# UM-Applied-Algorithms-Lab/AWRY

Measured on AMD Instinct MI355X. Metric: k-mer count queries/sec (parallel_count, random 31-mers, index resident in HBM), higher is better.
Workload: dtype u64

## Files before the change

awry_amd/_lib.py:

```python
import ctypes as C
import importlib.util
import os
import re

_HERE = os.path.dirname(os.path.abspath(__file__))
_SO = os.path.join(_HERE, "lib", "libawry_hip.so")
_HEADER = os.path.join(os.path.dirname(_HERE), "include", "awry_hip.h")
_lib = None


def lib_path():
    return _SO


class Pos(C.Structure):
    _fields_ = [("seq_idx", C.c_uint64), ("local_pos", C.c_uint64)]


class Range(C.Structure):
    _fields_ = [("start_ptr", C.c_uint64), ("end_ptr", C.c_uint64)]


class Anchor(C.Structure):
    _fields_ = [("q_begin", C.c_uint32), ("q_len", C.c_uint32), ("start_row", C.c_uint64), ("count", C.c_uint64)]
# ... 57 lines not shown

def load_library():
    global _lib
    if _lib is not None:
        return _lib
    if not os.path.exists(_SO):
        raise ImportError(
            "libawry_hip.so is not built (%s).  Run `python -m awry_amd.build` (needs hipcc); "
            "there is no CPU fallback for the search path." % _SO)
    _preload_hip_runtime()
    L = C.CDLL(_SO)
    vp, u64, u8, i32, cp = C.c_void_p, C.c_uint64, C.c_uint8, C.c_int, C.c_char_p
    u64p, u8p = C.POINTER(C.c_uint64), C.POINTER(C.c_uint8)
    vpp = C.POINTER(vp)

    def sig(name, res, *args):
        f = getattr(L, name)
        f.restype, f.argtypes = res, list(args)

    sig("awry_last_error", cp)
    sig("awry_build", i32, C.POINTER(BuildArgs), vpp)
    sig("awry_build_from_text", i32, vp, u64, i32, u64, u8, u64p, C.POINTER(cp), u64, vpp)
    sig("awry_build_from_text_on", i32, vp, u64, i32, u64, u8, u64p, C.POINTER(cp), u64, i32, vpp)
    sig("awry_load", i32, cp, vpp)
    sig("awry_save", i32, vp, cp)
    sig("awry_free", None, vp)
    sig("awry_set_devices", i32, vp, C.POINTER(i32), i32)
    sig("awry_set_seed_kmer_len", i32, vp, i32)
    sig("awry_seed_kmer_len", i32, vp)
    sig("awry_debug_set_count_kernel", i32, i32)
    sig("awry_debug_force_wide_rows", i32, i32)
    sig("awry_debug_set_max_blocks", i32, i32)
    sig("awry_debug_max_blocks", i32)
    sig("awry_debug_dense_sa", vp, vp, i32)
    sig("awry_debug_accelerators", i32, vp, i32, C.POINTER(DebugAccel))
    sig("awry_debug_seed_rung", vp, vp, i32, i32)
    sig("awry_debug_set_ctx_extra_cap", i32, i32)
    sig("awry_count_schedule", cp, vp, i32)
    sig("awry_num_devices", i32, vp)
    sig("awry_replica_device", i32, vp, i32)
    sig("awry_count_batch", i32, vp, vp, u64p, u64, u64p)
    sig("awry_count_packed_kmers", i32, vp, u64p, u64, i32, u64p)
    sig("awry_locate_batch", i32, vp, vp, u64p, u64, C.POINTER(u64p), C.POINTER(C.POINTER(Pos)), C.POINTER(u64p))
    sig("awry_free_buffer", None, vp)
    sig("awry_count_mismatch_batch", i32, vp, vp, u64p, u64, i32, u64p)
    sig("awry_locate_mismatch_batch", i32, vp, vp, u64p, u64, i32, C.POINTER(u64p), C.POINTER(C.POINTER(Pos)), C.POINTER(u64p),
        C.POINTER(u8p))
    sig("awry_dev_count_mismatch", i32, vp, i32, vp, vp, u64, i32, vp, vp, vp)
    sig("awry_dev_count_mismatch_tally", i32, vp, i32, vp, vp, u64, i32, vp, vp, vp, vp)
    u32 = C.c_uint32
    sig("awry_pattern_class", u32, i32, u8)
    sig("awry_count_pattern_batch", i32, vp, vp, u64p, u64, i32, u64p)
    sig("awry_locate_pattern_batch", i32, vp, vp, u64p, u64, i32, C.POINTER(u64p), C.POINTER(C.POINTER(Pos)), C.POINTER(u64p),
        C.POINTER(u8p))
    sig("awry_dev_count_pattern", i32, vp, i32, vp, vp, u64, i32, vp, vp, vp)
    sig("awry_dev_count_pattern_tally", i32, vp, i32, vp, vp, u64, i32, vp, vp, vp, vp)
    app = C.POINTER(C.POINTER(Anchor))
    sig("awry_anchor_batch", i32, vp, vp, u64p, u64, u32, i32, C.POINTER(u64p), app)
    sig("awry_locate_anchors_batch", i32, vp, vp, u64p, u64, u32, i32, u64, C.POINTER(u64p), app, C.POINTER(u64p),
        C.POINTER(C.POINTER(Pos)), C.POINTER(u64p))
    sig("awry_dev_anchors", i32, vp, i32, vp, vp, u64, u32, i32, vp, vp, vp, vp, vp)
    sig("awry_dev_anchors_tally", i32, vp, i32, vp, vp, u64, u32, i32, vp, vp, vp, vp, vp, vp)
    sig("awry_smem_batch", i32, vp, vp, u64p, u64, u32, C.POINTER(u64p), app)
    sig("awry_locate_smems_batch", i32, vp, vp, u64p, u64, u32, u64, C.POINTER(u64p), app, C.POINTER(u64p), C.POINTER(C.POINTER(Pos)), C.POINTER(u64p))
    sig("awry_dev_smems", i32, vp, i32, vp, vp, u64, u32, vp, vp, vp, vp, vp)
    sig("awry_dev_smems_tally", i32, vp, i32, vp, vp, u64, u32, vp, vp, vp, vp, vp, vp)
# ... 96 lines not shown
```

awry_amd/csrc/awry_hip.hip:

```cpp
#include "dev_common.h"
#include "replica.h"
#include "accelerators.h"
#include "launchers.h"
#include "host_count.h"
#include "host_locate.h"
#include "batch_host.h"
#include "mismatch_host.h"
#include "anchor_host.h"
#include "chain_host.h"
#include "edit_host.h"
#include "chain_align_host.h"
#include "map_host.h"
#include "pair_host.h"
#include "prewarm.h"

namespace {

template <class T>
T* malloc_array(size_t n) {
  const size_t bytes = std::max<size_t>(1, n) * sizeof(T);
  void* p = nullptr;
  if (bytes >= (8u << 20)) {
    if (posix_memalign(&p, 2u << 20, bytes) != 0) p = nullptr;
    if (p) (void)madvise(p, bytes, MADV_HUGEPAGE);
// ... 190 lines not shown
    idx->reps.clear();
    std::vector<std::unique_ptr<Replica>> reps(n_devices);
    if (n_devices == 1) {
      reps[0] = make_replica(idx, device_ids[0]);
    } else {
      std::vector<std::exception_ptr> errs(n_devices);
      std::vector<std::thread> pool;
      for (int i = 0; i < n_devices; i++)
        pool.emplace_back([&, i] {
          try { reps[i] = make_replica(idx, device_ids[i]); } catch (...) { errs[i] = std::current_exception(); }
        });
      for (auto& t : pool) t.join();
      for (auto& e : errs) if (e) std::rethrow_exception(e);
    }
    idx->reps = std::move(reps);
    for (auto& r : idx->reps) prewarm_host_paths(*r);
  });
}

int awry_set_seed_kmer_len(awry_index_t* idx, int k) {
  return guarded([&] {
    require(idx != nullptr, "null index");
    require(k >= -1 && k <= 17, "seed k-mer length must be in -1..17 (amino: ..7)");
    idx->seed_k_request = k;
    for (size_t s = 0; s < idx->reps.size(); s++) {
      Replica& r = replica(idx, (int)s);
      build_seed(idx, r, k < 0 ? default_seed_k(idx->host) : k);
      sync_seed_mode(idx, r);
    }
  });
}

int awry_debug_set_count_kernel(int mode) { g_count_kernel.store(mode); return AWRY_OK; }
int awry_debug_force_wide_rows(int on) { g_force_wide.store(on ? 1 : 0); return AWRY_OK; }
int awry_debug_set_max_blocks(int blocks) {
  if (blocks < 0) { g_last_error = "awry_debug_set_max_blocks: negative bound"; return AWRY_ERR_ARG; }
  g_max_blocks.store(blocks);
  return AWRY_OK;
}
int awry_debug_max_blocks(void) { return g_max_blocks.load(); }

const char* awry_count_schedule(const awry_index_t* idx, int L) {
  if (!idx || idx->reps.empty()) return "";
  const CountFacts f = count_facts(*idx->reps[0]);
  const uint64_t n = 1u << 20;
  return plan_name(L > 32 ? plan_reads(f, n, L, true, false) : plan_kmers(f, n, L, true, false));
}

int awry_seed_kmer_len(const awry_index_t* idx) { return idx && !idx->reps.empty() ? idx->reps[0]->seed_k : 0; }
int awry_num_devices(const awry_index_t* idx) { return idx ? (int)idx->reps.size() : 0; }
int awry_replica_device(const awry_index_t* idx, int slot) {
  return idx && slot >= 0 && slot < (int)idx->reps.size() ? idx->reps[slot]->device : -1;
}

int awry_count_batch(awry_index_t* idx, const uint8_t* qbytes, const uint64_t* qoff, uint64_t n, uint64_t* counts_out) {
  return guarded([&] {
    require(idx && qoff && (counts_out || n == 0), "null argument");
    require(qbytes || qoff[n] == qoff[0], "null query bytes");
    const auto t0 = std::chrono::steady_clock::now();
    for_each_replica(idx, n, [&](Replica& r, Shard sh, int) { count_shard(r, qbytes, qoff, sh, counts_out); });
    if (getenv("AWRY_TRACE_HOST"))
      fprintf(stderr, "[awry] awry_count_batch %.2f ms\n", std::chrono::duration<double, std::milli>(std::chrono::steady_clock::now() - t0).count());
  });
}

int awry_count_packed_kmers(awry_index_t* idx, const uint64_t* words, uint64_t n, int L, uint64_t* counts_out) {
// ... 1031 lines not shown
```

awry_amd/csrc/kernels.hip.h:

```cpp
#pragma once
#include <hip/hip_runtime.h>

#include "alphabet.h"
#include "layout.h"

#include "kernels_rank.hip.h"
#include "kernels_scan.hip.h"
#include "kernels_count.hip.h"
#include "kernels_anchor.hip.h"
#include "kernels_smem.hip.h"
#include "kernels_aa_kmer.hip.h"
#include "kernels_quad.hip.h"
#include "lcx.hip.h"
#include "kernels_nt2_kmer.hip.h"
#include "kmer_table.hip.h"
#include "kernels_seed.hip.h"
#include "kernels_pack.hip.h"
#include "kernels_reads.hip.h"
#include "lcx_kernels.hip.h"
#include "kernels_wide.hip.h"

namespace awry {

constexpr int LOC_TILE = 1024;
constexpr int LOC_QCAP = 1024;

constexpr uint64_t LOC_WALK_FLAG = 1ull << 63;

__device__ __forceinline__ void localise(const DevIndex& ix, uint64_t g, uint64_t* __restrict__ out) {
  uint64_t a = 0, z = ix.nseq;
  if (ix.seq_bucket) {
    const uint64_t b = g >> ix.seq_bucket_shift;
    a = ix.seq_bucket[b];
    z = (uint64_t)ix.seq_bucket[b + 1] + 1;
  }
  while (z - a > 1) { uint64_t mid = (a + z) >> 1; if (ix.seq_starts[mid] <= g) a = mid; else z = mid; }
  out[0] = a;
// ... 409 lines not shown
```

awry_amd/csrc/kernels_reads.hip.h:

```cpp
#pragma once

namespace awry {

template <bool USE_SEED, bool VERIFY, bool LIST, bool RAGGED>
__device__ __forceinline__ void reads_body(const DevIndex& ix, const uint64_t* __restrict__ queries, uint64_t n, int L,
                                           uint64_t* __restrict__ counts, uint64_t* __restrict__ range_start,
                                           const uint32_t* __restrict__ list_q, const uint32_t* __restrict__ lens, bool allow_lcx,
                                           uint64_t r_start = ~0ull, uint64_t r_stride = 64) {
  const int l = threadIdx.x & 3;
  const uint64_t nquads = ((uint64_t)gridDim.x * blockDim.x) >> 2;
  uint64_t r = r_start == ~0ull ? threadIdx.x >> 2 : r_start;
  uint64_t q = LIST ? (r < n ? list_q[r] : 0) : ((uint64_t)blockIdx.x * blockDim.x + threadIdx.x) >> 2;
  const uint64_t* __restrict__ blocks = ix.blocks;
  const SeedEntry* __restrict__ seed = ix.seed;
  const uint32_t* __restrict__ dense = ix.dense_sa;
  const uint32_t* __restrict__ text4 = ix.text4;
  const int k = USE_SEED ? ix.seed_k : 1, W = (L + 31) / 32;
  const int verify_after = (int)ix.verify_after;
  const bool lcx = USE_SEED && VERIFY && ix.lcx_key != nullptr && allow_lcx;
  const uint32_t cA = (uint32_t)ix.prefix_sums[1], cC = (uint32_t)ix.prefix_sums[2], cG = (uint32_t)ix.prefix_sums[3],
                 cN = (uint32_t)ix.prefix_sums[4], cT = (uint32_t)ix.prefix_sums[5], cEnd = (uint32_t)ix.prefix_sums[6];
  bool have = LIST ? r < n : q < n, fresh = true;
  uint64_t w = 0;
  uint32_t sp = 1, ep = 0;
// ... 145 lines not shown
          out_count = (uint64_t)__popc(vmask);
          if (ep == sp && vmask) out_rs = (RS_SINGLE << RS_MODE_SHIFT) | ((uint64_t)vp - (uint64_t)i);
          else out_rs = ((cand_lcx ? RS_LCX : RS_MULTI) << RS_MODE_SHIFT) | (uint64_t)sp | ((uint64_t)i << 32) | ((uint64_t)vmask << 48);
          cand_lcx = false;
        }
      }
      if (finished) {
        if (l == 0 && !hole) {
          counts[q] = out_count;
          if (range_start) range_start[q] = out_rs;
        }
        if (LIST) {
          r += r_stride;
          have = r < n;
          q = have ? list_q[r] : 0;
        } else {
          q += nquads;
          have = q < n;
        }
        fresh = true;
        mode = 0;
      }
    }
  }
}

template <bool USE_SEED, bool VERIFY, bool LIST = false, bool RAGGED = false>
__global__ __launch_bounds__(256) void count_nt2_reads_kernel(DevIndex ix, const uint64_t* __restrict__ queries, uint64_t n, int L,
                                                              uint64_t* __restrict__ counts, uint64_t* __restrict__ range_start,
                                                              Nt2Survivors sv = Nt2Survivors{}, const uint32_t* __restrict__ lens = nullptr) {
  if (LIST) reads_body<USE_SEED, VERIFY, LIST, RAGGED>(ix, queries, (uint64_t)sv.count[blockIdx.x], L, counts, range_start, sv.q + (uint64_t)blockIdx.x * sv.cap, lens, true);
  else reads_body<USE_SEED, VERIFY, LIST, RAGGED>(ix, queries, n, L, counts, range_start, nullptr, lens, true);
}
template <bool RAGGED>
__global__ __launch_bounds__(256) void count_nt2_reads_pool_kernel(DevIndex ix, const uint64_t* __restrict__ queries, int L, uint64_t* __restrict__ counts,
                                                                   uint64_t* __restrict__ range_start, Nt2Survivors sv, const uint32_t* __restrict__ lens) {
  reads_body<true, true, true, RAGGED>(ix, queries, (uint64_t)sv.count[0], L, counts, range_start, sv.q, lens, false,
                                       ((uint64_t)blockIdx.x * blockDim.x + threadIdx.x) >> 2, ((uint64_t)gridDim.x * blockDim.x) >> 2);
}

template <bool RAGGED>
__global__ __launch_bounds__(256) void count_nt2_reads_probe_kernel(DevIndex ix, const uint64_t* __restrict__ queries, uint64_t n, int L,
                                                                    uint64_t* __restrict__ counts, uint64_t* __restrict__ range_start,
                                                                    Nt2Survivors sv, const uint32_t* __restrict__ lens) {
  constexpr int VQ = 192;
  __shared__ unsigned int s_count;
  __shared__ uint32_t s_vsp[4][VQ], s_vq[4][VQ];
  __shared__ uint8_t s_vn[4][VQ];
  __shared__ uint16_t s_vl[RAGGED ? 4 : 1][VQ];
  __shared__ uint64_t s_vw[4][3][VQ];
  if (threadIdx.x == 0) s_count = 0;
  if (blockIdx.x == 0 && threadIdx.x == 0 && sv.lf_count) *sv.lf_count = 0;
  __syncthreads();
  const int lane = threadIdx.x & 63, wv_id = threadIdx.x >> 6;
  const SeedEntry* __restrict__ seed = ix.seed;
  const int k = ix.seed_k, W = (L + 31) / 32;
  const bool pos = ix.seed_pos != 0;
  const int min_i0 = pos ? 1 : 3;
  const int cx = (int)ix.ctx_extra, clen = SEED_CTX_LEN + cx;
  const uint64_t kmask = (1ull << (2 * k)) - 1;
  const uint64_t stride = (uint64_t)gridDim.x * blockDim.x;
  const uint64_t lane_lt = (1ull << lane) - 1;
  const uint64_t region = (uint64_t)blockIdx.x * sv.cap;
  const bool stash = L - k <= 96;
  int vcount = 0;
  auto settle = [&](uint64_t q, uint64_t count, uint64_t rs) {
    counts[q] = count;
    if (range_start) range_start[q] = rs;
  };
  auto drain = [&](int base, int cnt) {
    uint32_t q[2], sp[2], nc[2], vp[2];
    bool on[2];
#pragma unroll
    for (int h = 0; h < 2; h++) {
      const int s = base + lane + 64 * h;
      on[h] = lane + 64 * h < cnt;
      q[h] = on[h] ? s_vq[wv_id][s] : 0;
      sp[h] = on[h] ? s_vsp[wv_id][s] : 0;
      nc[h] = on[h] ? s_vn[wv_id][s] : 0;
      vp[h] = on[h] ? ((pos && nc[h] == 1u) ? sp[h] : ix.dense_sa[sp[h]]) : 0;
    }
#pragma unroll
    for (int h = 0; h < 2; h++) {
      if (!on[h]) continue;
      const int i0 = (RAGGED ? (int)s_vl[RAGGED ? wv_id : 0][base + lane + 64 * h] : L) - k, nchunks = (i0 + 31) >> 5;
// ... 125 lines not shown
```

awry_amd/csrc/launchers.h:

```cpp
#pragma once

namespace {

std::atomic<int> g_count_kernel{-1};
int count_kernel_override() {
  int m = g_count_kernel.load();
  if (m >= 0) return m;
  const char* e = getenv("AWRY_COUNT_KERNEL");
  if (e && !strcmp(e, "strided")) return 0;
  if (e && !strcmp(e, "chunk")) return 1;
  if (e && !strcmp(e, "quad4")) return 2;
  if (e && !strcmp(e, "twophase")) return 3;
  return -1;
}

CountFacts count_facts(const Replica& r) {
  static const bool rungs_off = getenv("AWRY_SEED_RUNGS") && !strcmp(getenv("AWRY_SEED_RUNGS"), "0");
  static const bool table_off = getenv("AWRY_KMER_TABLE") && !strcmp(getenv("AWRY_KMER_TABLE"), "0");
  CountFacts f;
  f.alphabet = r.dev.alphabet;
  f.wide = r.wide;
  f.bwt_len = r.dev.bwt_len;
  f.seed_k = r.seed_k;
  f.seed = r.seed.p != nullptr;
  f.seed64 = r.dev.seed64 != nullptr;
  f.text4 = r.dev.text4 != nullptr;
  f.dense_ratio = r.dev.dense_ratio;
  f.lcx_key = r.dev.lcx_key != nullptr;
  f.kt_mode = r.kt_mode;
  f.verify_kmers = r.verify_kmers;
  f.num_cus = r.num_cus;
  for (int i = 0; i < 4; i++) f.probe_resume_per_cu[i] = r.probe_resume_per_cu[i];
  for (int i = 0; i < 2; i++) f.lcx_reads_grid[i] = r.lcx_reads_grid[i];
  f.forced = count_kernel_override();
  f.rungs_off = rungs_off;
  f.table_off = table_off;
  return f;
}
dim3 plan_grid(const Replica& r, const CountPlan& p, uint64_t n) {
  return dim3(p.blocks ? p.blocks : (unsigned)grid_for(r, n * p.items_per_query, 256));
}


void launch_pack_nt2(Replica& r, const uint8_t* d_ascii, const uint64_t* d_off, uint64_t base, uint64_t n, uint64_t total_bytes, int L, int W,
                     uint64_t* d_words, uint32_t* d_lens, unsigned long long* d_bad, hipStream_t s, uint32_t* d_bad_list = nullptr) {
  if (n == 0) return;
// ... 130 lines not shown
    });
  } else {
    require(p.schedule == CountSchedule::WIDE_SINGLE, "internal: not a wide-row schedule");
    with_flags(p.seeded, d_lens != nullptr, [&](auto S, auto R) {
      hipLaunchKernelGGL((count_nt2_wide_kernel<S(), R()>), gw, bw, 0, s, r.dev, d_words, n, L, d_counts, d_range_start, d_lens, d_tally);
    });
  }
  HIP_CHECK(hipGetLastError());
}

void launch_count_nt2_long(Replica& r, const uint64_t* d_words, uint64_t n, int L, uint64_t* d_counts, uint64_t* d_range_start,
                           bool use_seed, hipStream_t s, const uint32_t* d_lens = nullptr) {
  require(r.dev.alphabet == NUCLEOTIDE, "packed 2-bit queries need a nucleotide index");
  require(L >= 1 && L <= 1 << 20, "packed read length out of range");
  if (n == 0) return;
  const ScratchLock scratch_lock(r, s);
  const CountPlan p = plan_reads(count_facts(r), n, L, use_seed, d_lens != nullptr);
  const dim3 g(plan_grid(r, p, n)), b(256);
  switch (p.schedule) {
    case CountSchedule::WIDE_SINGLE:
    case CountSchedule::WIDE_TWO_PHASE:
      launch_count_nt2_wide(r, p, d_words, n, L, d_counts, d_range_start, s, d_lens, nullptr);
      return;
    case CountSchedule::READS_LISTS:
    case CountSchedule::READS_LANES: {
      const bool lanes = p.schedule == CountSchedule::READS_LANES;
      Nt2Survivors sv, fb;
      two_phase_lists(r, s, n, p.blocks, p.lcx_grid, &sv, &fb);
      if (!lanes) sv.w = sv.range = nullptr;
      with_flags(d_lens != nullptr, [&](auto R) {
        hipLaunchKernelGGL(count_nt2_reads_probe_kernel<R()>, g, b, 0, s, r.dev, d_words, n, L, d_counts, d_range_start, sv, d_lens);
        if (lanes) {
          hipLaunchKernelGGL(lcx_quad_reads_kernel<R()>, dim3(p.lcx_grid), b, 0, s, r.dev, d_words, L, d_counts, d_range_start, sv, fb, p.blocks, d_lens);
          hipLaunchKernelGGL(count_nt2_reads_pool_kernel<R()>, g, b, 0, s, r.dev, d_words, L, d_counts, d_range_start, fb, d_lens);
        } else hipLaunchKernelGGL((count_nt2_reads_kernel<true, true, true, R()>), g, b, 0, s, r.dev, d_words, n, L, d_counts, d_range_start, sv, d_lens);
      });
      break;
    }
    case CountSchedule::READS_SINGLE: {
      const Nt2Survivors none{};
      with_flags(p.seeded, p.verify, d_lens != nullptr, [&](auto S, auto V, auto R) {
        hipLaunchKernelGGL((count_nt2_reads_kernel<S(), V(), false, R()>), g, b, 0, s, r.dev, d_words, n, L, d_counts, d_range_start, none, d_lens);
      });
      break;
    }
    default: require(false, "internal: not a schedule for reads");
  }
  HIP_CHECK(hipGetLastError());
}

void launch_count_nt2(Replica& r, const uint64_t* d_words, uint64_t n, int L, uint64_t* d_counts, bool use_seed, hipStream_t s,
                      unsigned long long* d_tally = nullptr) {
  require(r.dev.alphabet == NUCLEOTIDE, "packed 2-bit queries need a nucleotide index");
  require(L >= 1 && L <= 32, "packed k-mer length must be in 1..32");
  if (n == 0) return;
  const ScratchLock scratch_lock(r, s);
  CountFacts f = count_facts(r);
  CountPlan p = plan_kmers(f, n, L, use_seed, d_tally != nullptr);
  DevIndex dv = r.dev;
  std::shared_lock<std::shared_mutex> kt_lock;
  if (p.rung) {
    if (const SeedEntry* t = seed_rung(r, L)) { dv.seed = t; dv.seed_k = L; dv.seed_pos = 0; dv.ctx_extra = 0; }
    else { f.rung_failed = true; p = plan_kmers(f, n, L, use_seed, d_tally != nullptr); }
  }
  if (p.table) {
    if (const Replica::KmerTable* kt = kmer_table(r, L, true, kt_lock)) { dv.kmer_tab = kt->tab.p; dv.kmer_tab_bits = kt->bits; }
    else { f.table_failed = true; p = plan_kmers(f, n, L, use_seed, d_tally != nullptr); }
// ... 348 lines not shown
```

awry_amd/fm_index.py:

```python
import ctypes as C
import os
from dataclasses import dataclass
from typing import Iterable, List, Optional, Sequence

import numpy as np

from . import _lib

NUCLEOTIDE, AMINO = 0, 1
BUILD_HOST, BUILD_AUTO = -1, -2


class SymbolAlphabet:
    Nucleotide = NUCLEOTIDE
    Amino = AMINO


class AwryError(RuntimeError):
    def __init__(self, code, msg):
        super().__init__("awry error %d: %s" % (code, msg))
        self.code = code


ERR_IO, ERR_FORMAT, ERR_INVALID_QUERY, ERR_HIP, ERR_OOM, ERR_ARG, ERR_NO_DEVICE = -1, -2, -3, -4, -5, -6, -7
# ... 873 lines not shown

    def dev_count_nt2_tally(self, d_words, n, L, d_counts, d_tally, use_seed=True, stream=None, slot=0):
        _check(self._L.awry_dev_count_nt2_tally(self._h, slot, d_words, n, L, d_counts, 1 if use_seed else 0, d_tally, stream))

    def dev_count_ascii(self, d_qbytes, d_qoff, n, d_counts, d_ranges=None, d_status=None, stream=None, slot=0):
        _check(self._L.awry_dev_count_ascii(self._h, slot, d_qbytes, d_qoff, n, d_counts, d_ranges, d_status, stream))

    def dev_count_ascii_for_locate(self, d_qbytes, d_qoff, n, d_counts, d_locate_words, d_status=None, stream=None, slot=0):
        _check(self._L.awry_dev_count_ascii_for_locate(self._h, slot, d_qbytes, d_qoff, n, d_counts, d_locate_words, d_status, stream))

    def dev_count_ascii_uniform(self, d_qbytes, n, length, d_counts, d_status=None, stream=None, slot=0):
        _check(self._L.awry_dev_count_ascii_uniform(self._h, slot, d_qbytes, n, length, d_counts, d_status, stream))

    def dev_count_ascii_uniform_tally(self, d_qbytes, n, length, d_counts, d_tally, stream=None, slot=0):
        _check(self._L.awry_dev_count_ascii_uniform_tally(self._h, slot, d_qbytes, n, length, d_counts, d_tally, stream))

    def dev_scan_counts(self, d_counts, n, d_hit_off, d_scratch, stream=None, slot=0):
        _check(self._L.awry_dev_scan_counts(self._h, slot, d_counts, n, d_hit_off, d_scratch, stream))

    def dev_scan_scratch_bytes(self, n) -> int:
        return int(self._L.awry_dev_scan_scratch_bytes(n))

    def dev_locate(self, d_ranges, d_hit_off, n, total, d_gpos, d_pos=None, stream=None, slot=0, range_stride=2):
        _check(self._L.awry_dev_locate(self._h, slot, d_ranges, range_stride, d_hit_off, n, total, d_gpos, d_pos, stream))

    def dev_locate_tally(self, d_ranges, d_hit_off, n, total, d_gpos, d_pos, d_tally, stream=None, slot=0, range_stride=2):
        _check(self._L.awry_dev_locate_tally(self._h, slot, d_ranges, range_stride, d_hit_off, n, total, d_gpos, d_pos, d_tally, stream))

    def dev_phase_marker(self, phase_id, stream=None, slot=0):
        _check(self._L.awry_dev_phase_marker(self._h, slot, phase_id, stream))

    def dev_count_nt2_long(self, d_words, n, L, d_counts, d_range_start=None, use_seed=True, stream=None, slot=0):
        _check(self._L.awry_dev_count_nt2_long(self._h, slot, d_words, n, L, d_counts, d_range_start, 1 if use_seed else 0, stream))

    def set_locate_sa_ratio(self, ratio: int):
        _check(self._L.awry_set_locate_sa_ratio(self._h, ratio))

    def locate_sa_ratio(self) -> int:
        return self._L.awry_locate_sa_ratio(self._h)

    def set_lcx(self, on: bool):
        _check(self._L.awry_set_lcx(self._h, 1 if on else 0))

    def lcx_enabled(self) -> bool:
        return bool(self._L.awry_lcx_enabled(self._h))

    def set_kmer_table(self, mode: int):
        _check(self._L.awry_set_kmer_table(self._h, mode))

    def kmer_table_info(self, slot=0) -> dict:
        info = (C.c_uint64 * 6)()
        _check(self._L.awry_kmer_table_info(self._h, slot, info))
        return {"length": int(info[0]), "entries": int(info[1]), "lines": int(info[2]), "overflowed_lines": int(info[3]),
                "bytes": int(info[4]), "build_ms": int(info[5]) / 1000.0}

    def debug_kmer_table(self, slot=0):
        L, bits = C.c_int(0), C.c_uint32(0)
        for _ in range(4):
            _check(self._L.awry_debug_kmer_table(self._h, slot, None, 0, C.byref(L), C.byref(bits)))
            if L.value == 0:
                return None
            want = bits.value
            tab = np.empty(16 << want, np.uint64)
            _check(self._L.awry_debug_kmer_table(self._h, slot, tab.ctypes.data, len(tab), C.byref(L), C.byref(bits)))
            if L.value == 0:
                return None
# ... 119 lines not shown
```

include/awry_hip.h:

```cpp
#ifndef AWRY_HIP_H
#define AWRY_HIP_H
#include <stddef.h>
#include <stdint.h>

#ifdef __cplusplus
extern "C" {
#endif

enum {
  AWRY_OK = 0,
  AWRY_ERR_IO = -1,
  AWRY_ERR_FORMAT = -2,
  AWRY_ERR_INVALID_QUERY = -3,
  AWRY_ERR_HIP = -4,
  AWRY_ERR_OOM = -5,
  AWRY_ERR_ARG = -6,
  AWRY_ERR_NO_DEVICE = -7
};

enum { AWRY_NUCLEOTIDE = 0, AWRY_AMINO = 1 };

typedef struct awry_index awry_index_t;

typedef struct { uint64_t seq_idx, local_pos; } awry_pos_t;

typedef struct { uint64_t start_ptr, end_ptr; } awry_range_t;

typedef struct {
  const char *input_path;
  const char *sa_tmp_path;
  uint64_t sa_ratio;
  uint8_t kmer_len;
  uint8_t alphabet;
  uint64_t max_query_len;
  uint8_t remove_tmp;
} awry_build_args_t;

int awry_build(const awry_build_args_t *args, awry_index_t **out);
int awry_build_from_text(const uint8_t *text, uint64_t bwt_len, int alphabet, uint64_t sa_ratio, uint8_t kmer_len,
                         const uint64_t *seq_starts, const char *const *headers, uint64_t nseq, awry_index_t **out);
enum { AWRY_BUILD_HOST = -1, AWRY_BUILD_AUTO = -2 };
int awry_build_from_text_on(const uint8_t *text, uint64_t bwt_len, int alphabet, uint64_t sa_ratio, uint8_t kmer_len,
                            const uint64_t *seq_starts, const char *const *headers, uint64_t nseq, int build_device,
                            awry_index_t **out);
int awry_load(const char *path, awry_index_t **out);
int awry_save(awry_index_t *idx, const char *path);
void awry_free(awry_index_t *idx);

int awry_set_devices(awry_index_t *idx, const int *device_ids, int n_devices);
int awry_set_seed_kmer_len(awry_index_t *idx, int k);
int awry_seed_kmer_len(const awry_index_t *idx);
int awry_debug_set_count_kernel(int mode);
int awry_debug_force_wide_rows(int on);
int awry_debug_set_max_blocks(int blocks);
int awry_debug_max_blocks(void);
const void *awry_debug_dense_sa(const awry_index_t *idx, int slot);
typedef struct {
  const void *seed;
  int32_t seed_k, seed_entry_bytes, seed_pos, ctx_extra;
  const void *dense_sa;
  uint64_t dense_ratio;
  const void *text4;
  uint64_t text4_words;
  const void *text8;
  const void *sa_nblock;
  uint64_t nblock_lo, nblock_hi;
  const void *lcx_inner;
  uint64_t lcx_inner_words;
  uint32_t lcx_off[8];
} awry_debug_accel_t;
int awry_debug_accelerators(const awry_index_t *idx, int slot, awry_debug_accel_t *out);
const void *awry_debug_seed_rung(awry_index_t *idx, int slot, int L);
int awry_debug_set_ctx_extra_cap(int cap);
const char *awry_count_schedule(const awry_index_t *idx, int L);
int awry_set_locate_sa_ratio(awry_index_t *idx, int ratio);
int awry_locate_sa_ratio(const awry_index_t *idx);
int awry_set_verify(awry_index_t *idx, int after_steps);
int awry_set_verify_kmers(awry_index_t *idx, int on);
int awry_verify_enabled(const awry_index_t *idx);
int awry_set_lcx(awry_index_t *idx, int on);
int awry_lcx_enabled(const awry_index_t *idx);
int awry_debug_lcx(const awry_index_t *idx, int slot, const void **d_keys, const void **d_rowpos);
int awry_set_kmer_table(awry_index_t *idx, int mode);
int awry_kmer_table_info(awry_index_t *idx, int slot, uint64_t *info);
int awry_debug_set_kmer_table_lines(uint64_t lines);
// ... 274 lines not shown
```

rust/awry-hip-sys/src/lib.rs:

```rust
#![allow(non_camel_case_types)]
use std::os::raw::{c_char, c_int, c_void};

pub const AWRY_OK: c_int = 0;
pub const AWRY_ERR_IO: c_int = -1;
pub const AWRY_ERR_FORMAT: c_int = -2;
pub const AWRY_ERR_INVALID_QUERY: c_int = -3;
pub const AWRY_ERR_HIP: c_int = -4;
pub const AWRY_ERR_OOM: c_int = -5;
pub const AWRY_ERR_ARG: c_int = -6;
pub const AWRY_ERR_NO_DEVICE: c_int = -7;
pub const AWRY_NUCLEOTIDE: c_int = 0;
pub const AWRY_AMINO: c_int = 1;
pub const AWRY_BUILD_HOST: c_int = -1;
pub const AWRY_BUILD_AUTO: c_int = -2;

#[repr(C)]
pub struct awry_index_t {
    _private: [u8; 0],
}

#[repr(C)]
#[derive(Clone, Copy, Debug, Default, PartialEq, Eq)]
pub struct awry_pos_t {
    pub seq_idx: u64,
// ... 113 lines not shown
    pub text4_words: u64,
    pub text8: *const c_void,
    pub sa_nblock: *const c_void,
    pub nblock_lo: u64,
    pub nblock_hi: u64,
    pub lcx_inner: *const c_void,
    pub lcx_inner_words: u64,
    pub lcx_off: [u32; 8],
}

#[repr(C)]
pub struct awry_build_args_t {
    pub input_path: *const c_char,
    pub sa_tmp_path: *const c_char,
    pub sa_ratio: u64,
    pub kmer_len: u8,
    pub alphabet: u8,
    pub max_query_len: u64,
    pub remove_tmp: u8,
}

#[link(name = "awry_hip")]
extern "C" {
    pub fn awry_build(args: *const awry_build_args_t, out: *mut *mut awry_index_t) -> c_int;
    pub fn awry_build_from_text(text: *const u8, bwt_len: u64, alphabet: c_int, sa_ratio: u64, kmer_len: u8, seq_starts: *const u64, headers: *const *const c_char, nseq: u64, out: *mut *mut awry_index_t) -> c_int;
    pub fn awry_build_from_text_on(text: *const u8, bwt_len: u64, alphabet: c_int, sa_ratio: u64, kmer_len: u8, seq_starts: *const u64, headers: *const *const c_char, nseq: u64, build_device: c_int, out: *mut *mut awry_index_t) -> c_int;
    pub fn awry_load(path: *const c_char, out: *mut *mut awry_index_t) -> c_int;
    pub fn awry_save(idx: *mut awry_index_t, path: *const c_char) -> c_int;
    pub fn awry_free(idx: *mut awry_index_t);
    pub fn awry_set_devices(idx: *mut awry_index_t, device_ids: *const c_int, n_devices: c_int) -> c_int;
    pub fn awry_set_seed_kmer_len(idx: *mut awry_index_t, k: c_int) -> c_int;
    pub fn awry_seed_kmer_len(idx: *const awry_index_t) -> c_int;
    pub fn awry_debug_set_count_kernel(mode: c_int) -> c_int;
    pub fn awry_debug_force_wide_rows(on: c_int) -> c_int;
    pub fn awry_debug_set_max_blocks(blocks: c_int) -> c_int;
    pub fn awry_debug_max_blocks() -> c_int;
    pub fn awry_debug_dense_sa(idx: *const awry_index_t, slot: c_int) -> *const c_void;
    pub fn awry_debug_accelerators(idx: *const awry_index_t, slot: c_int, out: *mut awry_debug_accel_t) -> c_int;
    pub fn awry_debug_seed_rung(idx: *mut awry_index_t, slot: c_int, L: c_int) -> *const c_void;
    pub fn awry_debug_set_ctx_extra_cap(cap: c_int) -> c_int;
    pub fn awry_count_schedule(idx: *const awry_index_t, L: c_int) -> *const c_char;
    pub fn awry_set_locate_sa_ratio(idx: *mut awry_index_t, ratio: c_int) -> c_int;
    pub fn awry_locate_sa_ratio(idx: *const awry_index_t) -> c_int;
    pub fn awry_set_verify(idx: *mut awry_index_t, after_steps: c_int) -> c_int;
    pub fn awry_set_verify_kmers(idx: *mut awry_index_t, on: c_int) -> c_int;
    pub fn awry_verify_enabled(idx: *const awry_index_t) -> c_int;
    pub fn awry_set_lcx(idx: *mut awry_index_t, on: c_int) -> c_int;
    pub fn awry_lcx_enabled(idx: *const awry_index_t) -> c_int;
    pub fn awry_debug_lcx(idx: *const awry_index_t, slot: c_int, d_keys: *mut *const c_void, d_rowpos: *mut *const c_void) -> c_int;
    pub fn awry_set_kmer_table(idx: *mut awry_index_t, mode: c_int) -> c_int;
    pub fn awry_kmer_table_info(idx: *mut awry_index_t, slot: c_int, info: *mut u64) -> c_int;
    pub fn awry_debug_set_kmer_table_lines(lines: u64) -> c_int;
    pub fn awry_debug_kmer_table(idx: *mut awry_index_t, slot: c_int, host_out: *mut u64, capacity_words: u64, L_out: *mut c_int, bits_out: *mut u32) -> c_int;
    pub fn awry_num_devices(idx: *const awry_index_t) -> c_int;
    pub fn awry_count_batch(idx: *mut awry_index_t, qbytes: *const u8, qoff: *const u64, n: u64, counts_out: *mut u64) -> c_int;
    pub fn awry_count_packed_kmers(idx: *mut awry_index_t, words: *const u64, n: u64, L: c_int, counts_out: *mut u64) -> c_int;
    pub fn awry_locate_batch(idx: *mut awry_index_t, qbytes: *const u8, qoff: *const u64, n: u64, hit_off_out: *mut *mut u64, hits_out: *mut *mut awry_pos_t, global_pos_out: *mut *mut u64) -> c_int;
    pub fn awry_count_mismatch_batch(idx: *mut awry_index_t, qbytes: *const u8, qoff: *const u64, n: u64, max_mismatches: c_int, counts_out: *mut u64) -> c_int;
    pub fn awry_locate_mismatch_batch(idx: *mut awry_index_t, qbytes: *const u8, qoff: *const u64, n: u64, max_mismatches: c_int, hit_off_out: *mut *mut u64, hits_out: *mut *mut awry_pos_t, global_pos_out: *mut *mut u64, mismatches_out: *mut *mut u8) -> c_int;
    pub fn awry_pattern_class(alphabet: c_int, ascii: u8) -> u32;
    pub fn awry_count_pattern_batch(idx: *mut awry_index_t, qbytes: *const u8, qoff: *const u64, n: u64, max_mismatches: c_int, counts_out: *mut u64) -> c_int;
    pub fn awry_locate_pattern_batch(idx: *mut awry_index_t, qbytes: *const u8, qoff: *const u64, n: u64, max_mismatches: c_int, hit_off_out: *mut *mut u64, hits_out: *mut *mut awry_pos_t, global_pos_out: *mut *mut u64, mismatches_out: *mut *mut u8) -> c_int;
    pub fn awry_anchor_batch(idx: *mut awry_index_t, qbytes: *const u8, qoff: *const u64, n: u64, min_len: u32, skip: c_int, anchor_off_out: *mut *mut u64, anchors_out: *mut *mut awry_anchor_t) -> c_int;
    pub fn awry_locate_anchors_batch(idx: *mut awry_index_t, qbytes: *const u8, qoff: *const u64, n: u64, min_len: u32, skip: c_int, max_hits: u64, anchor_off_out: *mut *mut u64, anchors_out: *mut *mut awry_anchor_t, hit_off_out: *mut *mut u64, hits_out: *mut *mut awry_pos_t, global_pos_out: *mut *mut u64) -> c_int;
    pub fn awry_smem_batch(idx: *mut awry_index_t, qbytes: *const u8, qoff: *const u64, n: u64, min_len: u32, smem_off_out: *mut *mut u64, smems_out: *mut *mut awry_anchor_t) -> c_int;
    pub fn awry_locate_smems_batch(idx: *mut awry_index_t, qbytes: *const u8, qoff: *const u64, n: u64, min_len: u32, max_hits: u64, smem_off_out: *mut *mut u64, smems_out: *mut *mut awry_anchor_t, hit_off_out: *mut *mut u64, hits_out: *mut *mut awry_pos_t, global_pos_out: *mut *mut u64) -> c_int;
// ... 88 lines not shown
```

Measured before the change: 39.82 billion.

## Resolve pooled read survivors by suffix-array binary search before LF fallback

Adds a pre-pass to the reads pool kernel. Four-lane quads binary-search the dense suffix array, comparing packed text against the query to settle surviving long reads directly. Only reads that bail (saturated seed, text boundary or N) fall through to the existing backward-search body. The aim is to replace many dependent rank/LF steps with fewer text comparisons. In exchange it adds an extra fence and a bounded grid with changed launch bounds, plus census counters and debug APIs.

```diff
diff --git a/awry_amd/_lib.py b/awry_amd/_lib.py
--- a/awry_amd/_lib.py
+++ b/awry_amd/_lib.py
@@ -113,6 +113,9 @@
     sig("awry_debug_force_wide_rows", i32, i32)
     sig("awry_debug_set_max_blocks", i32, i32)
     sig("awry_debug_max_blocks", i32)
+    sig("awry_debug_set_reads_sa_search", i32, i32)
+    sig("awry_debug_reads_sa_search", i32)
+    sig("awry_debug_reads_census", i32, vp, i32, vp, C.POINTER(C.c_uint64))
     sig("awry_debug_dense_sa", vp, vp, i32)
     sig("awry_debug_accelerators", i32, vp, i32, C.POINTER(DebugAccel))
     sig("awry_debug_seed_rung", vp, vp, i32, i32)
diff --git a/awry_amd/csrc/awry_hip.hip b/awry_amd/csrc/awry_hip.hip
--- a/awry_amd/csrc/awry_hip.hip
+++ b/awry_amd/csrc/awry_hip.hip
@@ -246,6 +246,31 @@
 }
 
 int awry_debug_set_count_kernel(int mode) { g_count_kernel.store(mode); return AWRY_OK; }
+int awry_debug_set_reads_sa_search(int mode) {
+  if (mode < -1 || mode > 1) { g_last_error = "awry_debug_set_reads_sa_search: mode must be -1 (default), 0 (off) or 1 (on)"; return AWRY_ERR_ARG; }
+  g_reads_sa_search.store(mode);
+  return AWRY_OK;
+}
+int awry_debug_reads_sa_search(void) { return reads_sa_search_on() ? 1 : 0; }
+int awry_debug_reads_census(awry_index_t* idx, int slot, void* stream, uint64_t* census) {
+  return guarded([&] {
+    require(idx != nullptr && census != nullptr, "null argument");
+    Replica& r = replica(idx, slot);
+    for (int j = 0; j < 4; j++) census[j] = 0;
+    auto add = [&](hipStream_t s) {
+      const ScratchLock scratch_lock(r, s);
+      Replica::SurvScratch* sc = surv_scratch(r, s);
+      if (!sc->fcount.p) return;
+      uint32_t c[8];
+      HIP_CHECK(hipMemcpyAsync(c, sc->fcount.p, sizeof c, hipMemcpyDeviceToHost, s));
+      HIP_CHECK(hipStreamSynchronize(s));
+      for (int j = 0; j < 4; j++) census[j] += c[SAS_CENSUS_TAKEN + j];
+    };
+    if (stream == AWRY_STREAM_HOST_LANES) {
+      for (hipStream_t ls : r.lane_stream) if (ls) add(ls);
+    } else add((hipStream_t)stream);
+  });
+}
 int awry_debug_force_wide_rows(int on) { g_force_wide.store(on ? 1 : 0); return AWRY_OK; }
 int awry_debug_set_max_blocks(int blocks) {
   if (blocks < 0) { g_last_error = "awry_debug_set_max_blocks: negative bound"; return AWRY_ERR_ARG; }
diff --git a/awry_amd/csrc/kernels.hip.h b/awry_amd/csrc/kernels.hip.h
--- a/awry_amd/csrc/kernels.hip.h
+++ b/awry_amd/csrc/kernels.hip.h
@@ -3,6 +3,7 @@
 
 #include "alphabet.h"
 #include "layout.h"
+#include "sa_search.h"
 
 #include "kernels_rank.hip.h"
 #include "kernels_scan.hip.h"
diff --git a/awry_amd/csrc/kernels_reads.hip.h b/awry_amd/csrc/kernels_reads.hip.h
--- a/awry_amd/csrc/kernels_reads.hip.h
+++ b/awry_amd/csrc/kernels_reads.hip.h
@@ -201,11 +201,131 @@
   if (LIST) reads_body<USE_SEED, VERIFY, LIST, RAGGED>(ix, queries, (uint64_t)sv.count[blockIdx.x], L, counts, range_start, sv.q + (uint64_t)blockIdx.x * sv.cap, lens, true);
   else reads_body<USE_SEED, VERIFY, LIST, RAGGED>(ix, queries, n, L, counts, range_start, nullptr, lens, true);
 }
+enum : int { SAS_CENSUS_TAKEN = 1, SAS_CENSUS_SETTLED = 2, SAS_CENSUS_BAIL_TEXT = 3, SAS_CENSUS_BAIL_SEED = 4 };
+
 template <bool RAGGED>
-__global__ __launch_bounds__(256) void count_nt2_reads_pool_kernel(DevIndex ix, const uint64_t* __restrict__ queries, int L, uint64_t* __restrict__ counts,
-                                                                   uint64_t* __restrict__ range_start, Nt2Survivors sv, const uint32_t* __restrict__ lens) {
-  reads_body<true, true, true, RAGGED>(ix, queries, (uint64_t)sv.count[0], L, counts, range_start, sv.q, lens, false,
-                                       ((uint64_t)blockIdx.x * blockDim.x + threadIdx.x) >> 2, ((uint64_t)gridDim.x * blockDim.x) >> 2);
+__device__ __forceinline__ bool reads_sa_search(const DevIndex& ix, const uint64_t* __restrict__ queries, uint64_t n, int L,
+                                                uint64_t* __restrict__ counts, uint64_t* __restrict__ range_start, uint32_t* list_q,
+                                                const uint32_t* __restrict__ lens, uint64_t r_start, uint64_t r_stride, bool search,
+                                                uint32_t* __restrict__ census) {
+  const int l = threadIdx.x & 3, lane = threadIdx.x & 63;
+  const SeedEntry* __restrict__ seed = ix.seed;
+  const uint32_t* __restrict__ dense = ix.dense_sa;
+  const uint32_t* __restrict__ text4 = ix.text4;
+  const int k = ix.seed_k, W = (L + 31) / 32;
+  const uint64_t text_end = ix.bwt_len;
+  uint32_t c_taken = 0, c_settled = 0, c_text = 0, c_seed = 0;
+  uint64_t r = r_start;
+  bool have = r < n, fresh = true;
+  uint32_t q = 0;
+  int Lq = 0;
+  uint64_t myq = 0;
+  SaSearch s{0, 0, 0, 0};
+  bool single = false;
+  auto lane_compare = [&](uint32_t p, int c, uint64_t qword) -> uint32_t {
+    const int j0 = 128 * c + 32 * l, m = Lq - j0 > 32 ? 32 : Lq - j0;
+    if (m <= 0) return 0u;
+    const uint64_t g = (uint64_t)p + (uint64_t)j0;
+    if (g >= text_end) return sas_lane_code(SAS_BAIL, l);
+    const Text20 t = *reinterpret_cast<const Text20*>(text4 + (g >> 3));
+    const int sh = 4 * (int)(g & 7);
+    const uint64_t a0 = (uint64_t)t.w[0] | ((uint64_t)t.w[1] << 32), a1 = (uint64_t)t.w[2] | ((uint64_t)t.w[3] << 32), a2 = t.w[4];
+    const uint64_t tlo = sh ? (a0 >> sh) | (a1 << (64 - sh)) : a0, thi = sh ? (a1 >> sh) | (a2 << (64 - sh)) : a1;
+    return sas_lane_code(sas_compare32(tlo, thi, qword, m), l);
+  };
+  auto compare_rest = [&](uint32_t p) -> uint32_t {
+    uint32_t out = SAS_EQUAL;
+    for (int c = 1; out == SAS_EQUAL && 128 * c < Lq; c++) {
+      const int wi = 4 * c + l;
+      out = sas_first_outcome(quad_sum(lane_compare(p, c, wi < W ? queries[(uint64_t)q * W + wi] : 0ull)));
+    }
+    return out;
+  };
+  while (__any(have)) {
+    if (have) {
+      bool next = false, settled = false;
+      uint64_t out_count = 0, out_rs = (RS_PLAIN << RS_MODE_SHIFT) | 1ull;
+      if (fresh) {
+        fresh = false;
+        q = list_q[r];
+        if (q == 0xFFFFFFFFu) next = true;
+        else {
+          c_taken++;
+          if (!search) next = true;
+          else {
+            Lq = RAGGED ? (int)lens[q] : L;
+            const uint64_t* qw = queries + (uint64_t)q * W;
+            myq = l < W ? qw[l] : 0ull;
+            int what = SAS_SEED_BAIL;
+            SeedEntry e{0u, 0u};
+            if (Lq >= k) {
+              e = seed[qw[0] & ((1ull << (2 * k)) - 1)];
+              what = sas_entry(e, Lq, k, ix.seed_pos);
+            }
+            if (what == SAS_SEED_BAIL) { c_seed++; next = true; }
+            else if (what == SAS_EMPTY) { settled = true; }
+            else if (what == SAS_WHOLE) { settled = true; out_count = seed_cnt(e); out_rs = (RS_PLAIN << RS_MODE_SHIFT) | (uint64_t)e.sp; }
+            else {
+              single = what == SAS_SINGLE;
+              sas_begin(s, single ? seed_position(e, (int)ix.ctx_extra) : e.sp, seed_cnt(e));
+            }
+          }
+        }
+      } else {
+        const bool shared = sas_shared(s), a0 = sas_active0(s), a1 = sas_active1(s);
+        const uint32_t m0 = a0 ? sas_pivot0(s) : sas_pivot1(s), m1 = a1 && !shared ? sas_pivot1(s) : m0;
+        const uint32_t p0 = single ? m0 : dense[m0], p1 = single ? m1 : dense[m1];
+        const uint32_t c0 = lane_compare(p0, 0, myq), c1 = lane_compare(p1, 0, myq);
+        uint32_t out0 = sas_first_outcome(quad_sum(c0)), out1 = sas_first_outcome(quad_sum(c1));
+        if (Lq > 128) {
+          if (out0 == SAS_EQUAL) out0 = compare_rest(p0);
+          if (out1 == SAS_EQUAL) out1 = m1 == m0 ? out0 : compare_rest(p1);
+        }
+        if (!sas_apply(s, out0, out1)) { c_text++; next = true; }
+        else if (sas_done(s)) {
+          settled = true;
+          out_count = sas_count(s);
+          if (out_count) out_rs = ((single ? RS_SINGLE : RS_PLAIN) << RS_MODE_SHIFT) | (uint64_t)sas_first_row(s);
+        }
+      }
+      if (settled) {
+        c_settled++;
+        if (l == 0) {
+          counts[q] = out_count;
+          if (range_start) range_start[q] = out_rs;
+          list_q[r] = 0xFFFFFFFFu;
+        }
+        next = true;
+      }
+      if (next) {
+        r += r_stride;
+        have = r < n;
+        fresh = true;
+      }
+    }
+  }
+  if (census) {
+    uint32_t v[4] = {c_taken, c_settled, c_text, c_seed};
+#pragma unroll
+    for (int j = 0; j < 4; j++) {
+      uint32_t x = l == 0 ? v[j] : 0u;
+      for (int d = 32; d >= 4; d >>= 1) x += __shfl_xor(x, d, 64);
+      if (lane == 0 && x) atomicAdd(&census[SAS_CENSUS_TAKEN + j], x);
+    }
+  }
+  return c_settled != 0u;
+}
+
+template <bool RAGGED>
+__global__ __launch_bounds__(256, RAGGED ? 1 : 8) void count_nt2_reads_pool_kernel(DevIndex ix, const uint64_t* __restrict__ queries, int L, uint64_t* __restrict__ counts,
+                                                                   uint64_t* __restrict__ range_start, Nt2Survivors sv, const uint32_t* __restrict__ lens,
+                                                                   int sa_search) {
+  const uint64_t n = (uint64_t)sv.count[0];
+  const uint64_t r_start = ((uint64_t)blockIdx.x * blockDim.x + threadIdx.x) >> 2, r_stride = ((uint64_t)gridDim.x * blockDim.x) >> 2;
+  const bool holes = reads_sa_search<RAGGED>(ix, queries, n, L, counts, range_start, sv.q, lens, r_start, r_stride,
+                                            sa_search != 0 && ix.dense_sa != nullptr && ix.text4 != nullptr && ix.dense_ratio == 1u, sv.count);
+  if (__any(holes)) __threadfence();
+  reads_body<true, true, true, RAGGED>(ix, queries, n, L, counts, range_start, sv.q, lens, false, r_start, r_stride);
 }
 
 template <bool RAGGED>
@@ -219,7 +339,7 @@
   __shared__ uint16_t s_vl[RAGGED ? 4 : 1][VQ];
   __shared__ uint64_t s_vw[4][3][VQ];
   if (threadIdx.x == 0) s_count = 0;
-  if (blockIdx.x == 0 && threadIdx.x == 0 && sv.lf_count) *sv.lf_count = 0;
+  if (blockIdx.x == 0 && threadIdx.x <= SAS_CENSUS_BAIL_SEED && sv.lf_count) sv.lf_count[threadIdx.x] = 0;
   __syncthreads();
   const int lane = threadIdx.x & 63, wv_id = threadIdx.x >> 6;
   const SeedEntry* __restrict__ seed = ix.seed;
diff --git a/awry_amd/csrc/launchers.h b/awry_amd/csrc/launchers.h
--- a/awry_amd/csrc/launchers.h
+++ b/awry_amd/csrc/launchers.h
@@ -12,6 +12,13 @@
   if (e && !strcmp(e, "quad4")) return 2;
   if (e && !strcmp(e, "twophase")) return 3;
   return -1;
+}
+
+std::atomic<int> g_reads_sa_search{-1};
+bool reads_sa_search_on() {
+  static const bool env_off = getenv("AWRY_READS_SA_SEARCH") && !strcmp(getenv("AWRY_READS_SA_SEARCH"), "0");
+  const int m = g_reads_sa_search.load();
+  return m >= 0 ? m != 0 : !env_off;
 }
 
 CountFacts count_facts(const Replica& r) {
@@ -208,7 +215,7 @@
         hipLaunchKernelGGL(count_nt2_reads_probe_kernel<R()>, g, b, 0, s, r.dev, d_words, n, L, d_counts, d_range_start, sv, d_lens);
         if (lanes) {
           hipLaunchKernelGGL(lcx_quad_reads_kernel<R()>, dim3(p.lcx_grid), b, 0, s, r.dev, d_words, L, d_counts, d_range_start, sv, fb, p.blocks, d_lens);
-          hipLaunchKernelGGL(count_nt2_reads_pool_kernel<R()>, g, b, 0, s, r.dev, d_words, L, d_counts, d_range_start, fb, d_lens);
+          hipLaunchKernelGGL(count_nt2_reads_pool_kernel<R()>, dim3((unsigned)bound_blocks(g.x)), b, 0, s, r.dev, d_words, L, d_counts, d_range_start, fb, d_lens, reads_sa_search_on() ? 1 : 0);
         } else hipLaunchKernelGGL((count_nt2_reads_kernel<true, true, true, R()>), g, b, 0, s, r.dev, d_words, n, L, d_counts, d_range_start, sv, d_lens);
       });
       break;
diff --git a/awry_amd/csrc/sa_search.h b/awry_amd/csrc/sa_search.h
--- /dev/null
+++ b/awry_amd/csrc/sa_search.h
@@ -0,0 +1,84 @@
+#pragma once
+#include <stdint.h>
+
+#include "layout.h"
+
+namespace awry {
+
+enum : uint32_t { SAS_EQUAL = 0, SAS_LESS = 1, SAS_GREATER = 2, SAS_BAIL = 3 };
+
+enum : int {
+  SAS_TAKE = 0,
+  SAS_EMPTY,
+  SAS_WHOLE,
+  SAS_SEED_BAIL,
+  SAS_SINGLE,
+};
+AWRY_HD int sas_entry(SeedEntry e, int L, int k, uint32_t seed_pos) {
+  if (L < k) return SAS_SEED_BAIL;
+  const uint32_t cnt = seed_cnt(e);
+  if (cnt == SEED_CNT_SAT) return SAS_SEED_BAIL;
+  if (cnt == 0u) return SAS_EMPTY;
+  if (cnt == 1u && seed_pos) return SAS_SINGLE;
+  return L == k ? SAS_WHOLE : SAS_TAKE;
+}
+
+AWRY_HD uint64_t sas_spread16(uint64_t x) {
+  x &= 0xFFFFFFFFull;
+  x = (x | (x << 16)) & 0x0000FFFF0000FFFFull;
+  x = (x | (x << 8)) & 0x00FF00FF00FF00FFull;
+  x = (x | (x << 4)) & 0x0F0F0F0F0F0F0F0Full;
+  x = (x | (x << 2)) & 0x3333333333333333ull;
+  return x;
+}
+
+AWRY_HD uint32_t sas_compare32(uint64_t tlo, uint64_t thi, uint64_t qword, int m) {
+  const uint64_t qlo = sas_spread16(qword), qhi = sas_spread16(qword >> 32);
+  const uint64_t mlo = m >= 16 ? ~0ull : ((1ull << (4 * m)) - 1);
+  const uint64_t mhi = m <= 16 ? 0ull : (m >= 32 ? ~0ull : ((1ull << (4 * (m - 16))) - 1));
+  const uint64_t dlo = (tlo ^ qlo) & mlo, dhi = (thi ^ qhi) & mhi;
+  if (!(dlo | dhi)) return SAS_EQUAL;
+  const uint64_t d = dlo ? dlo : dhi, t = dlo ? tlo : thi, q = dlo ? qlo : qhi;
+  const int sh = __builtin_ctzll(d) & ~3;
+  const uint32_t tn = (uint32_t)(t >> sh) & 15u, qn = (uint32_t)(q >> sh) & 15u;
+  if (tn > 3u) return SAS_BAIL;
+  return tn < qn ? SAS_LESS : SAS_GREATER;
+}
+
+AWRY_HD uint32_t sas_lane_code(uint32_t outcome, int l) { return outcome << (2 * l); }
+AWRY_HD uint32_t sas_first_outcome(uint32_t codes) {
+  if (!codes) return SAS_EQUAL;
+  return (codes >> (__builtin_ctz(codes) & ~1)) & 3u;
+}
+
+struct SaSearch {
+  uint32_t lo0, hi0, lo1, hi1;
+};
+AWRY_HD void sas_begin(SaSearch& s, uint32_t sp, uint32_t cnt) {
+  s.lo0 = s.lo1 = sp;
+  s.hi0 = s.hi1 = sp + cnt;
+}
+AWRY_HD bool sas_active0(const SaSearch& s) { return s.lo0 < s.hi0; }
+AWRY_HD bool sas_active1(const SaSearch& s) { return s.lo1 < s.hi1; }
+AWRY_HD bool sas_done(const SaSearch& s) { return !sas_active0(s) && !sas_active1(s); }
+AWRY_HD bool sas_shared(const SaSearch& s) { return s.lo0 == s.lo1 && s.hi0 == s.hi1; }
+AWRY_HD uint32_t sas_pivot0(const SaSearch& s) { return s.lo0 + ((s.hi0 - s.lo0) >> 1); }
+AWRY_HD uint32_t sas_pivot1(const SaSearch& s) { return s.lo1 + ((s.hi1 - s.lo1) >> 1); }
+AWRY_HD bool sas_apply(SaSearch& s, uint32_t out0, uint32_t out1) {
+  const bool a0 = sas_active0(s), a1 = sas_active1(s);
+  if ((a0 && out0 == SAS_BAIL) || (a1 && out1 == SAS_BAIL)) return false;
+  const uint32_t m0 = sas_pivot0(s), m1 = sas_pivot1(s);
+  if (a0) {
+    if (out0 == SAS_LESS) s.lo0 = m0 + 1;
+    else s.hi0 = m0;
+  }
+  if (a1) {
+    if (out1 == SAS_GREATER) s.hi1 = m1;
+    else s.lo1 = m1 + 1;
+  }
+  return true;
+}
+AWRY_HD uint32_t sas_first_row(const SaSearch& s) { return s.lo0; }
+AWRY_HD uint32_t sas_count(const SaSearch& s) { return s.lo1 - s.lo0; }
+
+}
diff --git a/awry_amd/fm_index.py b/awry_amd/fm_index.py
--- a/awry_amd/fm_index.py
+++ b/awry_amd/fm_index.py
@@ -929,6 +929,11 @@
 
     def dev_count_nt2_long(self, d_words, n, L, d_counts, d_range_start=None, use_seed=True, stream=None, slot=0):
         _check(self._L.awry_dev_count_nt2_long(self._h, slot, d_words, n, L, d_counts, d_range_start, 1 if use_seed else 0, stream))
+
+    def reads_census(self, stream=None, slot=0, host_lanes=False) -> dict:
+        c = (C.c_uint64 * 4)()
+        _check(self._L.awry_debug_reads_census(self._h, slot, C.c_void_p(-1) if host_lanes else stream, c))
+        return {"taken": int(c[0]), "settled": int(c[1]), "bail_text": int(c[2]), "bail_seed": int(c[3])}
 
     def set_locate_sa_ratio(self, ratio: int):
         _check(self._L.awry_set_locate_sa_ratio(self._h, ratio))
diff --git a/include/awry_hip.h b/include/awry_hip.h
--- a/include/awry_hip.h
+++ b/include/awry_hip.h
@@ -51,6 +51,10 @@
 int awry_set_seed_kmer_len(awry_index_t *idx, int k);
 int awry_seed_kmer_len(const awry_index_t *idx);
 int awry_debug_set_count_kernel(int mode);
+int awry_debug_set_reads_sa_search(int mode);
+int awry_debug_reads_sa_search(void);
+#define AWRY_STREAM_HOST_LANES ((void *)-1)
+int awry_debug_reads_census(awry_index_t *idx, int slot, void *stream, uint64_t *census);
 int awry_debug_force_wide_rows(int on);
 int awry_debug_set_max_blocks(int blocks);
 int awry_debug_max_blocks(void);
diff --git a/rust/awry-hip-sys/src/lib.rs b/rust/awry-hip-sys/src/lib.rs
--- a/rust/awry-hip-sys/src/lib.rs
+++ b/rust/awry-hip-sys/src/lib.rs
@@ -169,6 +169,9 @@
     pub fn awry_set_seed_kmer_len(idx: *mut awry_index_t, k: c_int) -> c_int;
     pub fn awry_seed_kmer_len(idx: *const awry_index_t) -> c_int;
     pub fn awry_debug_set_count_kernel(mode: c_int) -> c_int;
+    pub fn awry_debug_set_reads_sa_search(mode: c_int) -> c_int;
+    pub fn awry_debug_reads_sa_search() -> c_int;
+    pub fn awry_debug_reads_census(idx: *mut awry_index_t, slot: c_int, stream: *mut c_void, census: *mut u64) -> c_int;
     pub fn awry_debug_force_wide_rows(on: c_int) -> c_int;
     pub fn awry_debug_set_max_blocks(blocks: c_int) -> c_int;
     pub fn awry_debug_max_blocks() -> c_int;
```

Result: slower. 39.13 billion (-1.7%).
